# febrianrachmadi/dep-gan-im

Hardware: AMD Instinct MI355X
Metric: 2D slices/sec (G+2D+GP train step), 256x256x1 fp32 (higher is better)
Workload: dtype f32; 1 GPU; DEP-GAN-IM twoCritics canonical train step (critic-Y2 + critic-DEM + G update, WGAN-GP), batch 32 per GPU, 256x256x1; per_gpu_batch=32, global_batch=32, parallelism=dp1

## Files before the change

### dep_gan_im_amd/csrc/igemm_wino.hip

```cpp
#include <stdlib.h>

#include <type_traits>

#include "common.h"
#include "epilogue.h"

namespace {

constexpr int WN_CK = 8;
constexpr int WN_TW = 18;
constexpr int WN_CP = 36;
constexpr int WN_XV = WN_CK / 4;

template <int MT>
struct WnCfg {
  static constexpr int TH = 8 * MT;
  static constexpr int NTILE = 32 * MT;
  static constexpr int PIXT = (TH + 2) * WN_TW;
  static constexpr int XTOT = PIXT * WN_XV;
  static constexpr int NXP = (XTOT + 255) / 256;
  static constexpr int RAW = NXP * 256 * 4;
  static_assert(XTOT % 4 == 0 && WN_TW % 2 == 0, "rslot permutes inside aligned groups of four slots: halo and padding stay apart");
  static constexpr int ZPLANE = NTILE * WN_CP + 32;
  static constexpr int Z = 8 * ZPLANE;
  static constexpr size_t LDS = sizeof(float) * (size_t)((2 * RAW) > Z ? (2 * RAW) : Z);
  static constexpr int WGS_PER_CU = (MT == 2) ? 2 : 3;
};

static __device__ __forceinline__ int rslot(int pix, int half) { return (2 * pix + half) ^ (((pix % WN_TW) >> 2) & 3); }
static __device__ __forceinline__ int rslot_inv(int q) { return q ^ ((((q >> 1) % WN_TW) >> 2) & 3); }

template <int MT, bool PERS, bool HEAD, int ABL = 0>
static __device__ __forceinline__ void wino_body(const ConvArgs& a) {
  typedef WnCfg<MT> C;
  constexpr int MF = 32, NT = 32;
  constexpr int WN_RAW = C::RAW, WN_ZPLANE = C::ZPLANE, WN_XTOT = C::XTOT, NXP = C::NXP;
  typedef f32x16 acc_t;
  extern __shared__ __attribute__((aligned(16))) float smem[];
  float* const raw0 = smem;
  float* const raw1 = smem + WN_RAW;

  const int tid = threadIdx.x;
  const int lane = tid & 63, wv = tid >> 6;
  const int r = lane & 31, h = lane >> 5;
  const int tilesX = (a.W + 15) >> 4, tilesY = (a.H + C::TH - 1) / C::TH;
  const unsigned nNTall = (unsigned)a.lgy, nPix = (unsigned)a.lgx;
  const int nCC = a.Cin / WN_CK;

  constexpr int SENT = (int)0x80000000;
  int xvo[NXP], xyx[NXP];
#pragma unroll
  for (int i = 0; i < NXP; ++i) {
    const int q = tid + i * 256;
    const int lq = rslot_inv(q);
    const int pix = lq >> 1, part = lq & 1;
    const int ly = pix / WN_TW, lx = pix - ly * WN_TW;
    xvo[i] = (q < WN_XTOT) ? 4 * (ly * (int)a.in.sY + lx * (int)a.in.sX + part * 4) : SENT;
    xyx[i] = (ly << 8) | lx;
  }
  int tA[MT][4], tB[MT][4];
  float tS[MT];
#pragma unroll
  for (int i = 0; i < MT; ++i) {
    const int cg = h, aa = wv, T = 32 * i + r;
    const int tyi = T >> 3, txi = T & 7;
    const int rA = (aa == 0) ? 0 : (aa == 2 ? 2 : 1), rB = (aa == 3) ? 3 : (aa == 2 ? 1 : 2);
#pragma unroll
    for (int j = 0; j < 4; ++j) {
      tA[i][j] = 4 * rslot((2 * tyi + rA) * WN_TW + 2 * txi + j, cg);
      tB[i][j] = 4 * rslot((2 * tyi + rB) * WN_TW + 2 * txi + j, cg);
    }
    tS[i] = (aa == 1) ? 1.f : -1.f;
  }
  const int wbase = __builtin_amdgcn_readfirstlane(wv * 256);
  const int boff = (4 * wv * 32 + r) * WN_CK + 4 * h;

  unsigned id = blockIdx.x;
  do {
    int t, ntile;
    if ((nPix & 7u) == 0) {
      const unsigned x = id & 7u, sl = id >> 3;
      ntile = (int)(sl % nNTall);
      t = (int)(x * (nPix >> 3) + sl / nNTall);
    } else {
      t = (int)(id % nPix);
      ntile = (int)(id / nPix);
    }
    const int tx0 = (t % tilesX) * 16;
    t /= tilesX;
    const int ty0 = (t % tilesY) * C::TH;
    const int b = t / tilesY;
    const long out_goff = 0;
    const int n0 = ntile * NT;
    const float* inb = a.in.p + (long)b * a.in.sB;
    const bool interior = ty0 >= 1 && ty0 + C::TH + 1 <= a.H && tx0 >= 1 && tx0 + 17 <= a.W;
    const char* halo0 = reinterpret_cast<const char*>(inb + ((long)(ty0 - 1) * a.in.sY + (long)(tx0 - 1) * a.in.sX));
    auto coff = [&](int cc) -> long {
      if (a.cpt > 0) {
        const int run = cc / a.cpt;
        return a.in_run_off[run] + (long)(cc - run * a.cpt) * WN_CK;
      }
      return (long)cc * WN_CK;
    };
    const float* const xorg = a.in.p - ((long)a.in.sY + (long)a.in.sX);
    const unsigned long long xu = (unsigned long long)xorg;
    const unsigned xlo = __builtin_amdgcn_readfirstlane((unsigned)xu), xhi = __builtin_amdgcn_readfirstlane((unsigned)(xu >> 32));
    const __amdgpu_buffer_rsrc_t rx =
        __builtin_amdgcn_make_buffer_rsrc((void*)(((unsigned long long)xhi << 32) | xlo), 0, 0x7FFFFFFF, 0x00020000);
    const int xso0 = 4 * (b * (int)a.in.sB + ty0 * (int)a.in.sY + tx0 * (int)a.in.sX);
    auto stage_dma = [&](int cc, int buf) {
      const int xso = xso0 + 4 * (int)coff(cc);
      float* xs = (buf ? raw1 : raw0) + wbase;
      if (interior) {
#pragma unroll
        for (int i = 0; i < NXP; ++i) {
          const int vo = xvo[i];
          __builtin_amdgcn_raw_ptr_buffer_load_lds(rx, (__attribute__((address_space(3))) void*)(xs + i * 1024), 16, vo,
                                                   xso, 0, 0);
        }
      } else {
#pragma unroll
        for (int i = 0; i < NXP; ++i) {
          const int iy = ty0 + (xyx[i] >> 8) - 1, ix = tx0 + (xyx[i] & 255) - 1;
          const int vo = (iy >= 0 && iy < a.H && ix >= 0 && ix < a.W) ? xvo[i] : SENT;
          __builtin_amdgcn_raw_ptr_buffer_load_lds(rx, (__attribute__((address_space(3))) void*)(xs + i * 1024), 16, vo,
                                                   xso, 0, 0);
        }
      }
    };

    acc_t acc[4][MT];

    const float* wnt = a.w + (size_t)ntile * nCC * (16 * NT * WN_CK) + boff;
    if (!(ABL & 8)) stage_dma(0, 0);
    auto chunk = [&](const int cc, auto first_tag) {
      constexpr bool FIRST = decltype(first_tag)::value;
      f32x4 bq[4];
#pragma unroll
      for (int f = 0; f < 4; ++f)
        bq[f] = *reinterpret_cast<const f32x4*>(wnt + (size_t)cc * (16 * NT * WN_CK) + f * (NT * WN_CK));
      asm volatile("s_waitcnt vmcnt(0)" ::: "memory");
      __syncthreads();
      if (!(ABL & 8) && cc + 1 < nCC) stage_dma(cc + 1, (cc + 1) & 1);
      const float* raw = (cc & 1) ? raw1 : raw0;
      f32x2 vr[MT][4][2];
      if (ABL & 2) {
#pragma unroll
        for (int i = 0; i < MT; ++i)
#pragma unroll
          for (int bb = 0; bb < 4; ++bb) vr[i][bb][0] = vr[i][bb][1] = f32x2{0.f, 0.f};
      }
#pragma unroll
      for (int i = 0; i < ((ABL & 2) ? 0 : MT); ++i) {
        const f32x2 s2 = {tS[i], tS[i]};
        f32x2 tc[4][2];
        f32x4 xs[4], ys[4];
#pragma unroll
        for (int j = 0; j < 4; ++j) {
          xs[j] = *reinterpret_cast<const f32x4*>(raw + tA[i][j]);
          ys[j] = *reinterpret_cast<const f32x4*>(raw + tB[i][j]);
        }
        __builtin_amdgcn_sched_barrier(0);
#pragma unroll
        for (int j = 0; j < 4; ++j) {
          const f32x4 x = xs[j], y = ys[j];
          tc[j][0] = __builtin_elementwise_fma(f32x2{y[0], y[1]}, s2, f32x2{x[0], x[1]});
          tc[j][1] = __builtin_elementwise_fma(f32x2{y[2], y[3]}, s2, f32x2{x[2], x[3]});
        }
#pragma unroll
        for (int p = 0; p < 2; ++p) {
          vr[i][0][p] = tc[0][p] - tc[2][p];
          vr[i][1][p] = tc[1][p] + tc[2][p];
          vr[i][2][p] = tc[2][p] - tc[1][p];
          vr[i][3][p] = tc[1][p] - tc[3][p];
        }
      }
#pragma unroll
      for (int f = 0; f < 4; ++f) {
        __builtin_amdgcn_sched_barrier(0);
#pragma unroll
        for (int j = 0; j < 4; ++j)
#pragma unroll
          for (int mt = 0; mt < MT; ++mt)
            if (!(ABL & 4)) {
              if (FIRST && j == 0) {
                const acc_t zero = {0.f, 0.f, 0.f, 0.f, 0.f, 0.f, 0.f, 0.f, 0.f, 0.f, 0.f, 0.f, 0.f, 0.f, 0.f, 0.f};
                acc[f][mt] = __builtin_amdgcn_mfma_f32_32x32x2f32(bq[f][j], vr[mt][f][j >> 1][j & 1], zero, 0, 0, 0);
              } else {
                acc[f][mt] = __builtin_amdgcn_mfma_f32_32x32x2f32(bq[f][j], vr[mt][f][j >> 1][j & 1], acc[f][mt], 0, 0, 0);
              }
            } else {
              if (FIRST && j == 0) acc[f][mt] = acc_t{};
              acc[f][mt][j] += bq[f][j] * vr[mt][f][j >> 1][j & 1];
            }
        __builtin_amdgcn_sched_barrier(0);
      }
    };
    chunk(0, std::true_type{});
    for (int cc = 1; cc < nCC; ++cc) chunk(cc, std::false_type{});

    if (ABL & 1) {
      float sacc = 0.f;
#pragma unroll
      for (int f = 0; f < 4; ++f)
#pragma unroll
        for (int mt = 0; mt < MT; ++mt)
#pragma unroll
          for (int j = 0; j < 16; ++j) sacc += acc[f][mt][j];
      if (sacc == 12345.678f) a.out.p[tid] = sacc;
      __syncthreads();
      continue;
    }
    auto zstage = [&]() {
      __syncthreads();
      float* zw = smem + (2 * wv) * WN_ZPLANE + r * WN_CP + 4 * h;
#pragma unroll
      for (int mt = 0; mt < MT; ++mt)
#pragma unroll
        for (int g = 0; g < 4; ++g) {
          f32x4 z0, z1;
#pragma unroll
          for (int k = 0; k < 4; ++k) {
            const float m0 = acc[0][mt][4 * g + k], m1 = acc[1][mt][4 * g + k], m2 = acc[2][mt][4 * g + k],
                        m3 = acc[3][mt][4 * g + k];
            z0[k] = (m0 + m1) + m2;
            z1[k] = (m1 - m2) - m3;
          }
          *reinterpret_cast<f32x4*>(zw + mt * (32 * WN_CP) + 8 * g) = z0;
          *reinterpret_cast<f32x4*>(zw + WN_ZPLANE + mt * (32 * WN_CP) + 8 * g) = z1;
        }
      __syncthreads();
    };
#define EPI_PRE_SYNC
#define EPI_STAGE
#define EPI_STAGE_LATE zstage()
#define EPI_NPASS (4 * MT)
#define EPI_OYW (ty0 + 2 * MT * __builtin_amdgcn_readfirstlane(wv))
#define EPI_FULL ((ty0 + C::TH <= a.H) && (tx0 + 16 <= a.W))
#define EPI_FETCH(v, py, px)                                                                                         \
  {                                                                                                                  \
    const float* zb = smem + ((px)&1) * WN_ZPLANE +                                                                  \
                      ((MT * __builtin_amdgcn_readfirstlane(wv) + ((py) >> 1)) * 8 + ((px) >> 1)) * WN_CP + c4;       \
    const f32x4 za = *reinterpret_cast<const f32x4*>(zb + (((py)&1) ? 2 : 0) * WN_ZPLANE);                           \
    const f32x4 zb1 = *reinterpret_cast<const f32x4*>(zb + (((py)&1) ? 4 : 2) * WN_ZPLANE);                          \
    const f32x4 zc = *reinterpret_cast<const f32x4*>(zb + (((py)&1) ? 6 : 4) * WN_ZPLANE);                           \
    _Pragma("unroll") for (int k_ = 0; k_ < 4; ++k_) v[k_] = ((py)&1) ? (za[k_] - zb1[k_]) - zc[k_] : (za[k_] + zb1[k_]) + zc[k_]; \
  }
#define EPI_HEAD HEAD
#include "igemm_epilogue.inc"
#undef EPI_HEAD
#undef EPI_FETCH
#undef EPI_FULL
#undef EPI_OYW
#undef EPI_NPASS
#undef EPI_STAGE_LATE
#undef EPI_STAGE
#undef EPI_PRE_SYNC
    if (PERS) __syncthreads();
  } while (PERS && (id += gridDim.x) < nPix * nNTall);
}

template <int MT, bool PERS>
__global__ __launch_bounds__(256, WnCfg<MT>::WGS_PER_CU) void wino_conv_kernel(const ConvArgs a) {
  wino_body<MT, PERS, false>(a);
}
template <bool PERS>
__global__ __launch_bounds__(256, 2) void wino_conv_head_kernel(const ConvArgs a) {
  wino_body<2, PERS, true>(a);
}
#ifdef DEPGAN_WINO_ABLATIONS
template <int MT, int ABL>
__global__ __launch_bounds__(256, WnCfg<MT>::WGS_PER_CU) void wino_conv_abl_kernel(const ConvArgs a) {
  wino_body<MT, true, false, ABL>(a);
}
#endif

}

bool dg_conv_wino_supported(const ConvPlan& pl, const ConvArgs& a) {
  if (!dg_plan_wino(pl)) return false;
  if (a.Cin != pl.Cin || (a.Cin % WN_CK) || (a.Cout % 32) || a.groups > 1 || a.dbg || ((a.H | a.W) & 1)) return false;
  if (a.cpt > 0 && ((a.Cin % (a.cpt * WN_CK)) != 0 || a.Cin / (a.cpt * WN_CK) > 4)) return false;
  return true;
}

static int wino_mt(const ConvArgs& a) {
  static int forced = -1;
  if (forced < 0) {
    const char* e = getenv("DEPGAN_WINO_MT");
    forced = e ? atoi(e) : 0;
  }
  if (a.ep.head_out) return 2;
  if (forced == 1 || forced == 2) return forced;
  return 1;
}

template <int MT>
static void wino_geometry(ConvArgs& a, long* total, long* G, bool* pers) {
  a.lgx = cdiv(a.W, 16) * cdiv(a.H, WnCfg<MT>::TH) * a.B;
  a.lgy = a.Cout / 32;
  *total = (long)a.lgx * a.lgy;
  const long cap = (long)WnCfg<MT>::WGS_PER_CU * dg_cu_count();
  *pers = *total > cap;
  *G = *pers ? cap : *total;
}

const char* dg_conv_wino_name(const ConvArgs& a_in) {
  ConvArgs a = a_in;
  long total, G;
  bool pers;
  const int mt = wino_mt(a);
  if (mt == 2) wino_geometry<2>(a, &total, &G, &pers); else wino_geometry<1>(a, &total, &G, &pers);
  if (a.ep.head_out) return pers ? "wino_conv_head_kernel<true>" : "wino_conv_head_kernel<false>";
  if (mt == 2) return pers ? "wino_conv_kernel<2,true>" : "wino_conv_kernel<2,false>";
  return pers ? "wino_conv_kernel<1,true>" : "wino_conv_kernel<1,false>";
}

template <int MT>
static int wino_launch(ConvArgs a, hipStream_t st) {
  long total, G;
  bool pers;
  wino_geometry<MT>(a, &total, &G, &pers);
  constexpr size_t LDS = WnCfg<MT>::LDS;
  static DgOncePerDevice once;
  if (once.need()) {
    HIPCHECK(hipFuncSetAttribute(reinterpret_cast<const void*>(&wino_conv_kernel<MT, false>),
                                 hipFuncAttributeMaxDynamicSharedMemorySize, (int)LDS));
    HIPCHECK(hipFuncSetAttribute(reinterpret_cast<const void*>(&wino_conv_kernel<MT, true>),
                                 hipFuncAttributeMaxDynamicSharedMemorySize, (int)LDS));
    if (MT == 2) {
      HIPCHECK(hipFuncSetAttribute(reinterpret_cast<const void*>(&wino_conv_head_kernel<false>),
                                   hipFuncAttributeMaxDynamicSharedMemorySize, (int)LDS));
      HIPCHECK(hipFuncSetAttribute(reinterpret_cast<const void*>(&wino_conv_head_kernel<true>),
                                   hipFuncAttributeMaxDynamicSharedMemorySize, (int)LDS));
    }
  }
#ifdef DEPGAN_WINO_ABLATIONS
  if (const char* e = getenv("DEPGAN_WINO_ABL")) {
    const int abl = atoi(e);
    if (abl && pers && !a.ep.head_out) {
#define WN_ABL_CASE(N)                                                                                              \
  case N:                                                                                                           \
    HIPCHECK(hipFuncSetAttribute(reinterpret_cast<const void*>(&wino_conv_abl_kernel<MT, N>),                       \
                                 hipFuncAttributeMaxDynamicSharedMemorySize, (int)LDS));                            \
    hipLaunchKernelGGL((wino_conv_abl_kernel<MT, N>), dim3((unsigned)G), dim3(256), LDS, st, a);                    \
    break;
      switch (abl) {
        WN_ABL_CASE(1) WN_ABL_CASE(2) WN_ABL_CASE(3) WN_ABL_CASE(4) WN_ABL_CASE(8) WN_ABL_CASE(10) WN_ABL_CASE(11)
        default: dg_set_error("DEPGAN_WINO_ABL=%d not instantiated", abl); return DG_ERR_ARG;
      }
      HIPCHECK(hipGetLastError());
      return DG_OK;
    }
  }
#endif
  if (a.ep.head_out) {
    if (MT != 2 || a.Cout != 32 || a.ep.pool.p) {
      dg_set_error("dg_conv_wino: the fused head needs 32 output channels and no fused pool");
      return DG_ERR_ARG;
    }
    if (pers) hipLaunchKernelGGL((wino_conv_head_kernel<true>), dim3((unsigned)G), dim3(256), LDS, st, a);
    else hipLaunchKernelGGL((wino_conv_head_kernel<false>), dim3((unsigned)G), dim3(256), LDS, st, a);
  } else {
    if (pers) hipLaunchKernelGGL((wino_conv_kernel<MT, true>), dim3((unsigned)G), dim3(256), LDS, st, a);
    else hipLaunchKernelGGL((wino_conv_kernel<MT, false>), dim3((unsigned)G), dim3(256), LDS, st, a);
  }
  HIPCHECK(hipGetLastError());
  return DG_OK;
}

int dg_conv_wino(const ConvPlan& pl, const ConvArgs& a, hipStream_t st) {
  if (!dg_conv_wino_supported(pl, a)) {
    dg_set_error("dg_conv_wino: shape not covered (3x3, Cin %% 8, Cout %% 32, even H and W, no groups)");
    return DG_ERR_UNSUPPORTED;
  }
  return wino_mt(a) == 2 ? wino_launch<2>(a, st) : wino_launch<1>(a, st);
}
```

Baseline: 662.9 slices/s.

## Generalize Winograd input staging to an N-buffer ring with counted vmcnt waits

Replaces the fixed double buffer and full vmcnt(0) drain in the Winograd conv main loop with a configurable ring of NBUF raw buffers. Waits are counted so only the oldest stage is drained, and the weight fragment loads are issued via inline asm and waited on just before the MFMAs. This lets weight loads overlap the input transform and keeps the next chunk's DMA in flight. LDS sizing is now bound to the Z exchange area. NBUF stays at 2, so the gain mainly comes from the finer-grained waits, at the cost of fragile hand-written counter accounting.

New measurement: 673.1 slices/s, median of 6. +1.5%, better.

```diff
diff --git a/dep_gan_im_amd/csrc/igemm_wino.hip b/dep_gan_im_amd/csrc/igemm_wino.hip
--- a/dep_gan_im_amd/csrc/igemm_wino.hip
+++ b/dep_gan_im_amd/csrc/igemm_wino.hip
@@ -23,9 +23,26 @@
   static_assert(XTOT % 4 == 0 && WN_TW % 2 == 0, "rslot permutes inside aligned groups of four slots: halo and padding stay apart");
   static constexpr int ZPLANE = NTILE * WN_CP + 32;
   static constexpr int Z = 8 * ZPLANE;
-  static constexpr size_t LDS = sizeof(float) * (size_t)((2 * RAW) > Z ? (2 * RAW) : Z);
+  static constexpr int NBUF = 2;
+  static_assert(NBUF >= 2 && NBUF * RAW <= Z, "the raw ring must fit under the Z exchange: LDS and workgroups per CU unchanged");
+  static_assert((NBUF - 1) * NXP + 4 < 64, "counted waits: vmcnt is a 6-bit field");
+  static constexpr size_t LDS = sizeof(float) * (size_t)Z;
   static constexpr int WGS_PER_CU = (MT == 2) ? 2 : 3;
 };
+
+template <int N>
+static __device__ __forceinline__ void wn_wait_vm() {
+  asm volatile("s_waitcnt vmcnt(%0)" ::"n"(N) : "memory");
+}
+template <int NX, int Y>
+static __device__ __forceinline__ void wn_wait_younger(int y) {
+  if constexpr (Y == 0) {
+    wn_wait_vm<4>();
+  } else {
+    if (y >= Y) wn_wait_vm<NX * Y + 4>();
+    else wn_wait_younger<NX, Y - 1>(y);
+  }
+}
 
 static __device__ __forceinline__ int rslot(int pix, int half) { return (2 * pix + half) ^ (((pix % WN_TW) >> 2) & 3); }
 static __device__ __forceinline__ int rslot_inv(int q) { return q ^ ((((q >> 1) % WN_TW) >> 2) & 3); }
@@ -34,11 +51,10 @@
 static __device__ __forceinline__ void wino_body(const ConvArgs& a) {
   typedef WnCfg<MT> C;
   constexpr int MF = 32, NT = 32;
-  constexpr int WN_RAW = C::RAW, WN_ZPLANE = C::ZPLANE, WN_XTOT = C::XTOT, NXP = C::NXP;
+  constexpr int WN_RAW = C::RAW, WN_ZPLANE = C::ZPLANE, WN_XTOT = C::XTOT, NXP = C::NXP, NBUF = C::NBUF;
+  constexpr int NXI = (ABL & 8) ? 0 : NXP;
   typedef f32x16 acc_t;
   extern __shared__ __attribute__((aligned(16))) float smem[];
-  float* const raw0 = smem;
-  float* const raw1 = smem + WN_RAW;
 
   const int tid = threadIdx.x;
   const int lane = tid & 63, wv = tid >> 6;
@@ -67,8 +83,8 @@
     const int rA = (aa == 0) ? 0 : (aa == 2 ? 2 : 1), rB = (aa == 3) ? 3 : (aa == 2 ? 1 : 2);
 #pragma unroll
     for (int j = 0; j < 4; ++j) {
-      tA[i][j] = 4 * rslot((2 * tyi + rA) * WN_TW + 2 * txi + j, cg);
-      tB[i][j] = 4 * rslot((2 * tyi + rB) * WN_TW + 2 * txi + j, cg);
+      tA[i][j] = 16 * rslot((2 * tyi + rA) * WN_TW + 2 * txi + j, cg);
+      tB[i][j] = 16 * rslot((2 * tyi + rB) * WN_TW + 2 * txi + j, cg);
     }
     tS[i] = (aa == 1) ? 1.f : -1.f;
   }
@@ -110,7 +126,7 @@
     const int xso0 = 4 * (b * (int)a.in.sB + ty0 * (int)a.in.sY + tx0 * (int)a.in.sX);
     auto stage_dma = [&](int cc, int buf) {
       const int xso = xso0 + 4 * (int)coff(cc);
-      float* xs = (buf ? raw1 : raw0) + wbase;
+      float* xs = smem + buf * WN_RAW + wbase;
       if (interior) {
 #pragma unroll
         for (int i = 0; i < NXP; ++i) {
@@ -132,17 +148,33 @@
     acc_t acc[4][MT];
 
     const float* wnt = a.w + (size_t)ntile * nCC * (16 * NT * WN_CK) + boff;
-    if (!(ABL & 8)) stage_dma(0, 0);
-    auto chunk = [&](const int cc, auto first_tag) {
+    if (!(ABL & 8)) {
+#pragma unroll
+      for (int k = 0; k < NBUF - 1; ++k)
+        if (k < nCC) stage_dma(k, k);
+    }
+    auto chunk = [&](const int cc, const int slot, auto first_tag) {
       constexpr bool FIRST = decltype(first_tag)::value;
+      const bool issue = cc + NBUF - 1 < nCC;
       f32x4 bq[4];
-#pragma unroll
-      for (int f = 0; f < 4; ++f)
-        bq[f] = *reinterpret_cast<const f32x4*>(wnt + (size_t)cc * (16 * NT * WN_CK) + f * (NT * WN_CK));
-      asm volatile("s_waitcnt vmcnt(0)" ::: "memory");
-      __syncthreads();
-      if (!(ABL & 8) && cc + 1 < nCC) stage_dma(cc + 1, (cc + 1) & 1);
-      const float* raw = (cc & 1) ? raw1 : raw0;
+      {
+        const float* wp = wnt + (size_t)cc * (16 * NT * WN_CK);
+        static_assert(3 * NT * WN_CK * sizeof(float) < 4096, "immediate offsets of the fragment loads");
+        asm volatile(
+            "global_load_dwordx4 %0, %4, off\n\t"
+            "global_load_dwordx4 %1, %4, off offset:1024\n\t"
+            "global_load_dwordx4 %2, %4, off offset:2048\n\t"
+            "global_load_dwordx4 %3, %4, off offset:3072"
+            : "=&v"(bq[0]), "=&v"(bq[1]), "=&v"(bq[2]), "=&v"(bq[3])
+            : "v"(wp)
+            : "memory");
+        static_assert(NT * WN_CK * sizeof(float) == 1024, "the offsets above");
+      }
+      wn_wait_younger<NXI, NBUF - 2>(nCC - 1 - cc);
+      __builtin_amdgcn_s_barrier();
+      asm volatile("" ::: "memory");
+      if (issue && !(ABL & 8)) stage_dma(cc + NBUF - 1, slot ? slot - 1 : NBUF - 1);
+      const char* raw = reinterpret_cast<const char*>(smem + slot * WN_RAW);
       f32x2 vr[MT][4][2];
       if (ABL & 2) {
 #pragma unroll
@@ -175,6 +207,14 @@
           vr[i][3][p] = tc[1][p] - tc[3][p];
         }
       }
+#pragma unroll
+      for (int i = 0; i < MT; ++i)
+        asm volatile("" : "+v"(vr[i][0][0]), "+v"(vr[i][0][1]), "+v"(vr[i][1][0]), "+v"(vr[i][1][1]), "+v"(vr[i][2][0]),
+                          "+v"(vr[i][2][1]), "+v"(vr[i][3][0]), "+v"(vr[i][3][1]));
+      __builtin_amdgcn_sched_barrier(0);
+      if (issue) wn_wait_vm<NXI>();
+      else wn_wait_vm<0>();
+      asm volatile("" : "+v"(bq[0]), "+v"(bq[1]), "+v"(bq[2]), "+v"(bq[3])::"memory");
 #pragma unroll
       for (int f = 0; f < 4; ++f) {
         __builtin_amdgcn_sched_barrier(0);
@@ -196,8 +236,8 @@
         __builtin_amdgcn_sched_barrier(0);
       }
     };
-    chunk(0, std::true_type{});
-    for (int cc = 1; cc < nCC; ++cc) chunk(cc, std::false_type{});
+    chunk(0, 0, std::true_type{});
+    for (int cc = 1, s = 1 % NBUF; cc < nCC; ++cc, s = (s + 1 == NBUF) ? 0 : s + 1) chunk(cc, s, std::false_type{});
 
     if (ABL & 1) {
       float sacc = 0.f;
```
